# GT-RIPL/robo-vln

Measured on AMD Instinct MI355X. Metric: policy env-steps/sec (batched act()) at 256x256 RGB-D, 80-tok instr, higher is better.
Workload: dtype fp16 (range-calibrated fp16 storage and MFMA in BERT, both trunks and the cross-modal block; fp32 accumulate, fp32 recurrent state; DESIGN.md section 5); 1 GPU; BASELINE.json configs[1]: full HCM act() (hi->argmax->lo), 256x256 RGB-D, L=80, VLA N=1, LSTM-512; per_gpu_batch=64, global_batch=64, parallelism=single GPU

## Files before the change

### include/hcm.h

```cpp
#ifndef HCM_H
#define HCM_H

#include <stdint.h>

#ifdef __cplusplus
extern "C" {
#endif

typedef struct hcm_ctx* hcm_handle;

enum hcm_status {
    HCM_OK = 0,
    HCM_ERR_ARG = -1,
    HCM_ERR_STATE = -2,
    HCM_ERR_KEY = -3,
    HCM_ERR_SHAPE = -4,
    HCM_ERR_HIP = -5,
    HCM_ERR_UNSUPPORTED = -6,
    HCM_ERR_NOMEM = -7
};

enum hcm_dtype { HCM_F32 = 0, HCM_BF16 = 1, HCM_I32 = 2, HCM_I64 = 3, HCM_U8 = 4, HCM_F16 = 5 };
enum hcm_model { HCM_HIGH = 0, HCM_LOW = 1, HCM_CMA = 2 ,
                 HCM_S2S = 3  };
// ... 162 lines not shown


int hcm_debug_enable_taps(hcm_handle h, int enable);
int hcm_debug_get_tap(hcm_handle h, const char* name, float* host_out, int64_t capacity,
                      int64_t* n_out, int64_t* shape_out);
int hcm_debug_igemm_prof(uint64_t* out8, int reset);
int hcm_debug_gemm256_prof(uint64_t* out1024, int reset);
int hcm_debug_marks(hcm_handle h, uint64_t* out256, char* names, int names_cap);

int hcm_op_conv2d(const void* x, const void* w_ohwi, const float* bias, const void* residual, void* y,
                  int dtype, int B, int H, int W, int Cin, int Cout, int KH, int KW, int stride, int pad,
                  int act, void* stream);
int hcm_op_conv2d_gn(const void* x, const void* w_ohwi, const float* gamma, const float* beta, const void* residual, void* y,
                     int dtype, int B, int H, int W, int Cin, int Cout, int KH, int KW, int stride, int pad, int groups, float eps,
                     int relu, void* stream);
int hcm_op_bottleneck_tail(const void* x, const void* w2, const float* b2, const void* w3, const float* b3, const void* identity,
                           void* y, int dtype, int B, int H, int W, int C1, int stride, void* stream);
int hcm_op_bottleneck_tail_next(const void* x, const void* w2, const float* b2, const void* w3, const float* b3, const void* identity,
                                void* y, const void* w1, const float* b1, void* o1, int dtype, int B, int H, int W, int C1, int stride,
                                int CN, void* stream);
int hcm_op_bottleneck_tail_ds(const void* x, const void* w2, const float* b2, const void* w3ds, const float* b3ds, const void* xd,
                              void* y, const void* w1, const float* b1, void* o1, int dtype, int B, int H, int W, int stride,
                              void* stream);
int hcm_op_conv2d_gn_large(const void* x, const void* w_ohwi, const float* gamma, const float* beta, const void* residual, void* y,
                           int dtype, int B, int H, int W, int Cin, int Cout, int KH, int KW, int stride, int pad, int groups, float eps,
                           int relu, void* stream);
int hcm_op_stem_conv(const void* x, int x_dtype, const void* w, const float* bias, void* y, int dtype, int B, int H, int W, int C,
                     int Cout, int KH, int KW, int stride, int pad, int K, int Kp, int rowrun, float scale, int act, void* stream);
int hcm_op_stem_conv_packed(const void* x, int x_dtype, const void* w, const float* bias, void* y, int dtype, int B, int H, int W,
                            int Cout, float scale, int act, void* scratch, void* stream);
int hcm_op_stem_conv_packed_pool(const void* x, int x_dtype, const void* w, const float* bias, void* y, int dtype, int B, int H, int W,
                                 int Cout, float scale, void* scratch, void* half_map, void* stream);
int hcm_op_stem_pool_fused(const void* x, int x_dtype, const void* w, const float* bias, void* y, int dtype, int B, int H, int W,
                           int Cout, float scale, void* scratch, void* stream);
int hcm_op_stem_pool_fused_red(const void* x, int x_dtype, const void* w, const float* bias, void* y, int dtype, int B, int H, int W,
                               int Cout, float scale, void* scratch, const void* w1, const float* b1, void* o1, void* stream);
int64_t hcm_op_stem_scratch_bytes(int B, int H, int W);
int hcm_op_depth_conv8x8s4(const float* depth, const void* w, const float* bias, void* y, int dtype, int B, int H, int act, void* scratch,
                           void* stream);
int hcm_op_simplecnn3(const float* depth, const void* w0, const float* b0, const void* w1_frag, const float* b1, const void* w2_frag, const float* b2,
                      void* y, int dtype, int B, int H, void* stream);
int hcm_op_linear(const void* x, const void* w, const float* bias, const void* residual, void* y,
                  int dtype, int M, int N, int K, int act, int out_f32, void* stream);
int hcm_op_vla_layer(const void* q, const void* I, const void* const* kv, const int* Lk, const void* const* att, void* const* out, float* const* pooled,
                     int ld_pool, const void* wo, const float* bo, const void* w1, const float* b1, const void* w2, const float* b2, const float* g1,
                     const float* be1, const float* g2, const float* be2, const int32_t* lens, int dtype, int B, int L, int d_ff, int streams,
// ... 32 lines not shown
```

### robo-vln_amd/_lib.py

```python
import ctypes as C
import os

_HERE = os.path.dirname(os.path.abspath(__file__))
LIB_PATH = os.path.join(_HERE, "libhcm_dev.so" if os.environ.get("HCM_DEV_LIB", "0") not in ("", "0") else "libhcm.so")

HCM_F32, HCM_BF16, HCM_I32, HCM_I64, HCM_U8, HCM_F16 = 0, 1, 2, 3, 4, 5
HCM_HIGH, HCM_LOW, HCM_CMA, HCM_S2S = 0, 1, 2, 3
HCM_ENC_RESNET, HCM_ENC_SIMPLECNN = 0, 1
HCM_LSTM, HCM_GRU = 0, 1
(HCM_NUM_RECURRENT_LAYERS, HCM_HIDDEN_SIZE, HCM_NUM_ACTIONS, HCM_RECORD_WIDTH, HCM_WORKSPACE_BYTES,
 HCM_WEIGHT_BYTES, HCM_MAX_BATCH, HCM_GRAPH_LAUNCHES, HCM_EAGER_LAUNCHES, HCM_FP16_FALLBACK, HCM_CALIB_MAX_BERT, HCM_CALIB_MAX_DEPTH,
 HCM_CALIB_NONFINITE, HCM_CALIB_MAX_RGB, HCM_CALIB_MAX_VLA, HCM_STEP_NONFINITE, HCM_RANGE_FOLD, HCM_GATHER_JOINED) = range(18)
PRECISIONS = {"fp32": HCM_F32, "fp16": HCM_F16, "bf16": HCM_BF16}
ACT_NONE, ACT_RELU, ACT_GELU = 0, 1, 2
HCM_ACT_REUSE_INSTRUCTION = 1
HCM_ACT_HOST_FRAMES = 2
HCM_ACT_CHAIN_GRAPHS = 4

STATUS_EXC = {-1: ValueError, -2: RuntimeError, -3: KeyError, -4: ValueError, -5: RuntimeError, -6: ValueError,
              -7: MemoryError}


class HcmConfigStruct(C.Structure):
    _fields_ = [(n, C.c_int32) for n in (
# ... 50 lines not shown
                             C.c_void_p, C.c_void_p, C.c_void_p, C.c_void_p, C.c_void_p, C.c_void_p, C.c_int, C.c_void_p]),
    "hcm_comm_unique_id": (C.c_int, [C.c_void_p]),
    "hcm_comm_init": (C.c_int, [C.c_void_p, C.c_void_p, C.c_int, C.c_int]),
    "hcm_comm_abort": (C.c_int, [C.c_void_p]),
    "hcm_gather_poison": (C.c_int, [C.c_void_p, C.c_int, C.c_void_p, C.c_void_p, C.c_void_p]),
    "hcm_act_gather": (C.c_int, [C.c_void_p, C.c_void_p, C.c_int, C.c_void_p, C.c_void_p, C.c_int, C.c_void_p, C.c_int, C.c_int,
                                 C.c_void_p, C.c_void_p, C.c_void_p, C.c_void_p, C.c_void_p, C.c_void_p, C.c_int, C.c_void_p, C.c_void_p]),
    "hcm_refresh_instruction": (C.c_int, [C.c_void_p, C.c_void_p, C.c_int, C.c_void_p, C.c_int, C.c_int, C.POINTER(C.c_int32), C.c_int, C.c_void_p]),
    "hcm_calibrate": (C.c_int, [C.c_void_p, C.c_void_p, C.c_int, C.c_void_p, C.c_void_p, C.c_int, C.c_int, C.c_int, C.c_void_p]),
    "hcm_release_host_weights": (C.c_int, [C.c_void_p]),
    "hcm_query": (C.c_int, [C.c_void_p, C.c_int, C.POINTER(C.c_int64)]),
    "hcm_guard_poll": (C.c_int, [C.c_void_p, C.c_void_p, C.POINTER(C.c_int64)]),
    "hcm_last_error": (C.c_char_p, [C.c_void_p]),
    "hcm_destroy": (None, [C.c_void_p]),
    "hcm_debug_enable_taps": (C.c_int, [C.c_void_p, C.c_int]),
    "hcm_debug_get_tap": (C.c_int, [C.c_void_p, C.c_char_p, C.c_void_p, C.c_int64, C.POINTER(C.c_int64), C.POINTER(C.c_int64)]),
    "hcm_debug_igemm_prof": (C.c_int, [C.POINTER(C.c_uint64), C.c_int]),
    "hcm_debug_gemm256_prof": (C.c_int, [C.POINTER(C.c_uint64), C.c_int]),
    "hcm_debug_marks": (C.c_int, [C.c_void_p, C.POINTER(C.c_uint64), C.c_char_p, C.c_int]),
    "hcm_op_conv2d": (C.c_int, [C.c_void_p] * 5 + [C.c_int] * 11 + [C.c_void_p]),
    "hcm_op_bottleneck_tail": (C.c_int, [C.c_void_p] * 7 + [C.c_int] * 6 + [C.c_void_p]),
    "hcm_op_bottleneck_tail_next": (C.c_int, [C.c_void_p] * 10 + [C.c_int] * 7 + [C.c_void_p]),
    "hcm_op_bottleneck_tail_ds": (C.c_int, [C.c_void_p] * 10 + [C.c_int] * 5 + [C.c_void_p]),
    "hcm_op_conv2d_gn": (C.c_int, [C.c_void_p] * 6 + [C.c_int] * 11 + [C.c_float, C.c_int, C.c_void_p]),
    "hcm_op_conv2d_gn_large": (C.c_int, [C.c_void_p] * 6 + [C.c_int] * 11 + [C.c_float, C.c_int, C.c_void_p]),
    "hcm_op_stem_conv": (C.c_int, [C.c_void_p, C.c_int, C.c_void_p, C.c_void_p, C.c_void_p] + [C.c_int] * 13 + [C.c_float, C.c_int, C.c_void_p]),
    "hcm_op_stem_conv_packed": (C.c_int, [C.c_void_p, C.c_int, C.c_void_p, C.c_void_p, C.c_void_p] + [C.c_int] * 5 + [C.c_float, C.c_int, C.c_void_p, C.c_void_p]),
    "hcm_op_stem_pool_fused": (C.c_int, [C.c_void_p, C.c_int, C.c_void_p, C.c_void_p, C.c_void_p] + [C.c_int] * 5 + [C.c_float, C.c_void_p, C.c_void_p]),
    "hcm_op_stem_pool_fused_red": (C.c_int, [C.c_void_p, C.c_int, C.c_void_p, C.c_void_p, C.c_void_p] + [C.c_int] * 5 + [C.c_float] + [C.c_void_p] * 5),
    "hcm_op_stem_conv_packed_pool": (C.c_int, [C.c_void_p, C.c_int, C.c_void_p, C.c_void_p, C.c_void_p] + [C.c_int] * 5 + [C.c_float, C.c_void_p, C.c_void_p, C.c_void_p]),
    "hcm_op_depth_conv8x8s4": (C.c_int, [C.c_void_p] * 4 + [C.c_int] * 4 + [C.c_void_p, C.c_void_p]),
    "hcm_op_stem_scratch_bytes": (C.c_int64, [C.c_int] * 3),
    "hcm_op_linear": (C.c_int, [C.c_void_p] * 5 + [C.c_int] * 6 + [C.c_void_p]),
    "hcm_op_linear_impl": (C.c_int, [C.c_void_p] * 5 + [C.c_int] * 7 + [C.c_void_p]),
    "hcm_op_vla_layer": (C.c_int, [C.c_void_p] * 7 + [C.c_int] + [C.c_void_p] * 11 + [C.c_int] * 5 + [C.c_void_p]),
    "hcm_op_vla_layer_frag": (C.c_int, [C.c_void_p] * 7 + [C.c_int] + [C.c_void_p] * 11 + [C.c_int] * 5 + [C.c_void_p]),
    "hcm_op_attention": (C.c_int, [C.c_void_p] * 4 + [C.c_int] * 9 + [C.c_void_p]),
    "hcm_op_simplecnn3": (C.c_int, [C.c_void_p] * 8 + [C.c_int] * 3 + [C.c_void_p]),
    "hcm_op_pack_frag": (C.c_int, [C.c_void_p, C.c_void_p, C.c_int, C.c_int, C.c_int, C.c_void_p]),
    "hcm_op_bert_attn_block": (C.c_int, [C.c_void_p] * 9 + [C.c_int] * 3 + [C.c_void_p, C.c_float, C.c_void_p]),
    "hcm_op_layernorm": (C.c_int, [C.c_void_p] * 5 + [C.c_int] * 3 + [C.c_float, C.c_void_p]),
    "hcm_op_layernorm_post": (C.c_int, [C.c_void_p] * 5 + [C.c_int, C.c_void_p] + [C.c_int] * 3 + [C.c_float, C.c_void_p]),
    "hcm_op_groupnorm": (C.c_int, [C.c_void_p] * 4 + [C.c_int] * 5 + [C.c_float, C.c_int, C.c_void_p]),
    "hcm_op_conv2d_gn_pool": (C.c_int, [C.c_void_p] * 5 + [C.c_int] * 11 + [C.c_float, C.c_void_p]),
    "hcm_op_conv2d_gn_res2": (C.c_int, [C.c_void_p] * 9 + [C.c_int] * 9 + [C.c_float, C.c_int, C.c_void_p]),
    "hcm_op_val_loss": (C.c_int, [C.c_void_p] * 7 + [C.c_int] * 3 + [C.c_void_p]),
# ... 33 lines not shown
```

### robo-vln_amd/csrc/api.cpp

```cpp
#include <chrono>
#include <cmath>
#include <cstdlib>
#include <cstring>
#include <stdexcept>
#include <string>

#include "model.h"

namespace hcm {
void build_spec_high(hcm_ctx* ctx);
void build_spec_low(hcm_ctx* ctx);
void prepare_high(hcm_ctx* ctx);
void prepare_low(hcm_ctx* ctx);
void build_spec_cma(hcm_ctx* ctx);
void prepare_cma(hcm_ctx* ctx);
void run_refresh_instruction(hcm_ctx* ctx, const void* ids, int ids_dt, int B, const int32_t* idx, int n);
void run_cma(hcm_ctx* ctx, const void* rgb, int rgb_dt, const float* depth, const void* ids, int ids_dt, int B, const float* h_in,
             const float* mask, float* out, float* stop, float* h_out);
void build_spec_s2s(hcm_ctx* ctx);
void prepare_s2s(hcm_ctx* ctx);
void run_s2s(hcm_ctx* ctx, const void* rgb, int rgb_dt, const float* depth, const void* ids, int ids_dt, int B, int Bi, const float* h_in,
             const float* mask, float* out, float* stop, float* progress, float* h_out, int T = 1);
void comm_destroy(hcm_ctx* ctx);
void run_step(hcm_ctx* ctx, bool do_hi, bool do_lo, const void* rgb, int rgb_dt, const float* depth, const void* ids, int ids_dt,
// ... 1121 lines not shown
    return op_rc(launch_bneck23(b, op_dt(dtype), (hipStream_t)stream));
}
int hcm_op_bottleneck_tail_next(const void* x, const void* w2, const float* b2, const void* w3, const float* b3, const void* identity,
                                void* y, const void* w1, const float* b1, void* o1, int dtype, int B, int H, int W, int C1, int stride,
                                int CN, void* stream) {
    Bneck23 b;
    b.x = x; b.w2 = w2; b.b2 = b2; b.w3 = w3; b.b3 = b3; b.res = identity; b.y = y;
    b.B = B; b.H = H; b.W = W; b.C1 = C1; b.stride = stride;
    b.w1 = w1; b.b1 = b1; b.o1 = o1; b.CN = CN;
    if (!w1) return HCM_ERR_ARG;
    return op_rc(launch_bneck23(b, op_dt(dtype), (hipStream_t)stream));
}
int hcm_op_bottleneck_tail_ds(const void* x, const void* w2, const float* b2, const void* w3ds, const float* b3ds, const void* xd,
                              void* y, const void* w1, const float* b1, void* o1, int dtype, int B, int H, int W, int stride,
                              void* stream) {
    if (!xd || !w1) return HCM_ERR_ARG;
    Bneck23 b;
    b.x = x; b.w2 = w2; b.b2 = b2; b.w3 = w3ds; b.b3 = b3ds; b.y = y;
    b.B = B; b.H = H; b.W = W; b.C1 = 64; b.stride = stride;
    b.w1 = w1; b.b1 = b1; b.o1 = o1; b.CN = 64;
    b.xd = xd; b.xdC = 64; b.KD = 1;
    return op_rc(launch_bneck23(b, op_dt(dtype), (hipStream_t)stream));
}
int hcm_op_conv2d_gn(const void* x, const void* w_ohwi, const float* gamma, const float* beta, const void* residual, void* y,
                     int dtype, int B, int H, int W, int Cin, int Cout, int KH, int KW, int stride, int pad, int groups, float eps,
                     int relu, void* stream) {
    if (groups < 1 || Cout % groups) return HCM_ERR_ARG;
    IGemm g;
    g.x = x; g.w = w_ohwi; g.res = residual; g.y = y;
    g.B = B; g.H = H; g.W = W; g.Cin = Cin; g.xC = Cin;
    g.Ho = (H + 2 * pad - KH) / stride + 1; g.Wo = (W + 2 * pad - KW) / stride + 1;
    g.KH = KH; g.KW = KW; g.stride = stride; g.pad = pad;
    g.M = B * g.Ho * g.Wo; g.N = Cout; g.K = KH * KW * Cin; g.Kp = g.K; g.ldy = Cout; g.ldr = Cout; g.act = relu ? ACT_RELU : ACT_NONE;
    g.gn_gamma = gamma; g.gn_beta = beta; g.gn_cg = Cout / groups; g.gn_hw = g.Ho * g.Wo; g.gn_eps = eps;
    return op_rc(launch_igemm(g, op_dt(dtype), (hipStream_t)stream));
}
int hcm_op_stem_conv(const void* x, int x_dtype, const void* w, const float* bias, void* y, int dtype, int B, int H, int W, int C, int Cout,
                     int KH, int KW, int stride, int pad, int K, int Kp, int rowrun, float scale, int act, void* stream) {
    IGemm g;
    g.x = x; g.w = w; g.bias = bias; g.y = y;
    g.B = B; g.H = H; g.W = W; g.Cin = C; g.xC = C;
    g.Ho = (H + 2 * pad - KH) / stride + 1; g.Wo = (W + 2 * pad - KW) / stride + 1;
    g.KH = KH; g.KW = KW; g.stride = stride; g.pad = pad;
    g.M = B * g.Ho * g.Wo; g.N = Cout; g.K = K; g.Kp = Kp; g.ldy = Cout; g.ldr = Cout; g.act = act;
    g.x_src_dt = x_dtype == HCM_U8 ? DT_U8 : x_dtype == HCM_F32 ? DT_F32 : op_dt(x_dtype);
    g.x_scale = scale; g.x_rowrun = rowrun;
// ... 271 lines not shown
```

### robo-vln_amd/csrc/forward.cpp

```cpp
#include <cstdio>
#include <cstdlib>
#include <stdexcept>

#include "model.h"

namespace hcm {

int depth_final_spatial(const hcm_config& c);
int depth_compress_channels(const hcm_config& c);

struct Act { void* p = nullptr; int B = 0, H = 0, W = 0, C = 0; };

struct Fwd {
    hcm_ctx* ctx;
    Arena& ar;
    hipStream_t s;
    int dt;
    size_t esz;
    bool dry;

    explicit Fwd(hcm_ctx* c) : ctx(c), ar(c->arena), s(c->stream), dt(c->dt_vla), esz(dt_size(c->dt_vla)), dry(c->arena.dry) {}

    void use(int d) { dt = d; esz = dt_size(d); }

// ... 374 lines not shown
            int fr[3], nf = 0;
            if (pre >= 0) fr[nf++] = pre;
            for (int i = 0; i < 4; ++i) if (i != xi && i != pre) fr[nf++] = i;
            if (nf != 3) throw std::runtime_error("trunk slot rotation: expected three free activation slots");
            if (xpend.valid && xpend.res && slot[fr[0]] == xpend.res) std::swap(fr[0], fr[1]);
            void* sa = slot[fr[0]]; void* sb = slot[fr[1]]; void* sc = slot[fr[2]];
            if (xpend.valid && xpend.res && sa == xpend.res) throw std::runtime_error("trunk slot rotation: c1 would overwrite a pending identity");
            const int Ho2 = (x.H + 2 - 3) / b.stride + 1, Wo2 = (x.W + 2 - 3) / b.stride + 1;
            Act o1{sa, B, x.H, x.W, CO(b.c1)};
            const bool have_o1 = pre >= 0;
            pre = -1;
            Pending p1, p2;
            if (have_o1) {}
            else if (t.gn) {
                if (xpend.valid) { xpend.writeback = true; pend_in = xpend; xpend.valid = false; }
                defer_out = &p1;
                conv_gn(b.c1, x, sa, 1, 0, nullptr, b.n1, G, true, x.H, x.W);
            }
            else conv(b.c1, x, sa, 1, 0, nullptr, ACT_RELU, x.H, x.W);
            static const bool no_tail = dev_env("HCM_NO_BNECK_FUSE") != nullptr;
            static const bool no_next = dev_env("HCM_NO_BNECK_NEXT") != nullptr;
            static const bool no_256 = dev_env("HCM_NO_BNECK256") != nullptr;
            static const bool force_256 = dev_env("HCM_FORCE_BNECK256") != nullptr;
            const BottleneckW* nb = bi + 1 < t.blocks.size() ? &t.blocks[bi + 1] : nullptr;
            static const int next_only = dev_env("HCM_BNECK_NEXT_ONLY") ? atoi(dev_env("HCM_BNECK_NEXT_ONLY")) : 0;
            const bool next = nb && !no_next && (!next_only || next_only == b.c2.Cout) && nb->c1.KH == 1 && nb->c1.KW == 1 && nb->c1.Cin == b.c3.Cout && nb->c1.Kp == nb->c1.Cin &&
                              nb->c1.bias && nb->c1.groups == b.c2.groups && nb->c1.dt == b.c2.dt &&
                              ((nb->c1.Cout == b.c2.Cout && (nb->c1.Cout == 64 || nb->c1.Cout == 128 || nb->c1.Cout == 256)) || (b.c2.Cout == 64 && nb->c1.Cout == 128));
            const long tiles256 = (long)b.c2.groups * (((long)B * ((x.H + 2 - 3) / b.stride + 1) * ((x.W + 2 - 3) / b.stride + 1) + 127) / 128);
            const bool c1_ok = b.c2.Cout == 64 || b.c2.Cout == 128 || (b.c2.Cout == 256 && next && !no_256 && (tiles256 >= 192 || force_256));
            if (!t.gn && !no_tail && (b.c2.dt == DT_BF16 || b.c2.dt == DT_F16) && c1_ok && b.c2.KH == 3 &&
                b.c2.Cin == b.c2.Cout && b.c2.Kp == 9 * b.c2.Cin && b.c3.Cout == 4 * b.c2.Cout && b.c3.Kp == b.c2.Cout && b.c2.bias && b.c3.bias &&
                b.c3.groups == b.c2.groups) {
                const void* idt = x.p;
                static const bool no_dsfold = dev_env("HCM_NO_BNECK_DSFOLD") != nullptr;
                const bool dsfold = b.has_ds && !no_dsfold && next && b.c3ds.w && b.c2.Cout == 64 && nb->c1.Cout == 64 && b.ds.Cin == 64 &&
                                    b.c3ds.Kp == 128 && b.c3ds.groups == b.c2.groups && x.C == b.c2.groups * 64;
                if (b.has_ds && !dsfold) {
                    conv(b.ds, x, sb, b.stride, 0, nullptr, ACT_NONE, Ho2, Wo2);
                    idt = sb;
                }
                const int pre_slot = (b.has_ds && !dsfold) ? xi : fr[1];
                if (!dry) {
                    Bneck23 q;
                    q.x = sa; q.w2 = b.c2.w; q.b2 = b.c2.bias; q.w3 = b.c3.w; q.b3 = b.c3.bias; q.res = idt; q.y = sc;
                    q.B = B; q.H = x.H; q.W = x.W; q.C1 = b.c2.Cout; q.xC = o1.C; q.stride = b.stride;
                    q.ldy = q.ldr = CO(b.c3);
                    if (b.c2.groups > 1) {
                        q.groups = b.c2.groups; q.g_x = b.c2.Cin; q.g_w2 = (long long)b.c2.Cout * b.c2.Kp; q.g_b2 = b.c2.Cout;
                        q.g_w3 = (long long)b.c3.Cout * b.c3.Kp; q.g_b3 = b.c3.Cout; q.g_y = b.c3.Cout;
                    }
                    if (next) {
                        q.w1 = nb->c1.w; q.b1 = nb->c1.bias; q.o1 = slot[pre_slot]; q.CN = nb->c1.Cout; q.ldo = CO(nb->c1);
                        if (b.c2.groups > 1) { q.g_w1 = (long long)nb->c1.Cout * nb->c1.Kp; q.g_b1 = nb->c1.Cout; q.g_o1 = nb->c1.Cout; }
                    }
                    if (dsfold) {
                        q.w3 = b.c3ds.w; q.b3 = b.c3ds.bias; q.res = nullptr;
                        q.xd = x.p; q.xdC = x.C; q.KD = 1;
                        if (b.c2.groups > 1) { q.g_w3 = (long long)b.c3ds.Cout * b.c3ds.Kp; q.g_xd = 64; }
                    }
                    ck(launch_bneck23(q, b.c2.dt, s), "bottleneck tail");
                    calib_check(sc, b.c2.dt, B * Ho2 * Wo2, CO(b.c3), CO(b.c3));
                }
                if (next) pre = pre_slot;
                x = Act{sc, B, Ho2, Wo2, CO(b.c3)};
                xi = fr[2];
                ++bidx;
                if (bidx == 3 || bidx == 7 || bidx == 13 || bidx == 16) {
                    tap(tapname + "_layer" + std::to_string(bidx == 3 ? 1 : bidx == 7 ? 2 : bidx == 13 ? 3 : 4), x.p, true, {B, x.H, x.W, x.C});
                    mark(tapname + ".layer" + std::to_string(bidx == 3 ? 1 : bidx == 7 ? 2 : bidx == 13 ? 3 : 4) + "_end");
                }
                continue;
            }
            Act o2{sb, B, Ho2, Wo2, CO(b.c2)};
            if (t.gn) {
                pend_in = p1; p1.valid = false;
                defer_out = &p2;
                conv_gn(b.c2, o1, sb, b.stride, 1, nullptr, b.n2, G, true, Ho2, Wo2);
            }
            else conv(b.c2, o1, sb, b.stride, 1, nullptr, ACT_RELU, Ho2, Wo2);
            const void* idt = x.p;
            Pending pds;
// ... 1146 lines not shown
```

### robo-vln_amd/csrc/igemm.hip

```cpp
#include <cstdio>
#include <cstdlib>
#include <cstring>
#include <type_traits>
#include <vector>
#include <algorithm>
#include <mutex>
#include <string>
#include <unordered_map>
#include "kernels.h"
#include "dev.h"

namespace hcm {

typedef float f32x4 __attribute__((ext_vector_type(4)));
typedef __bf16 bf16x8 __attribute__((ext_vector_type(8)));

struct IGemmDev {
    const char* x; const char* w; const float* bias; const char* res; char* y;
    int B, H, W, Cin, xC, Ho, Wo, KH, KW, stride, pad;
    int stride_w;
    int M, N, K, Kp, ldy, ldr, act, out_f32;
    int image_epi;
    int res_f32;
    int cin_shift, kw_rcp, tilesM, tilesN, map;
// ... 3065 lines not shown
            g_choice[key] = choice;
        } else {
            choice = heuristic_choice(d, dt);
        }
    }
    static const bool log_shapes = dev_env("HCM_IGEMM_LOG") != nullptr;
    if (log_shapes) {
        static std::unordered_map<std::string, int> seen;
        std::lock_guard<std::mutex> l(g_choice_mu);
        if (seen.emplace(key, choice).second)
            fprintf(stderr, "[igemm] dt=%d M=%d N=%d K=%d groups=%d KHxKW=%dx%d stride=%d res=%d -> choice %d\n", dt, d.M, d.N, d.K, d.groups, d.KH, d.KW,
                    d.stride, d.res != nullptr, choice);
    }
    return launch_dt(d, dt, choice, s);
}


constexpr int kHaloRing = 5, kHaloRingD = 5;

hipError_t launch_bneck23(const Bneck23& b, int dt, hipStream_t s) {
    if (dt != DT_BF16 && dt != DT_F16) return hipErrorInvalidValue;
    if ((b.C1 != 64 && b.C1 != 128 && b.C1 != 256) || (!b.res && !b.xd) || !b.b2 || !b.b3 || b.stride < 1) return hipErrorInvalidValue;
    if (b.C1 == 256 && (!b.w1 || b.CN != 256 || b.xd)) return hipErrorInvalidValue;
    if (b.xd && (b.C1 != 64 || b.KD != 1 || !b.w1 || b.CN != 64 || (b.xdC % 8))) return hipErrorInvalidValue;
    const int C3 = 4 * b.C1;
    const int ldy = b.ldy ? b.ldy : C3, ldr = b.ldr ? b.ldr : C3, xC = b.xC ? b.xC : b.C1;
    if ((ldy % 8) || (ldr % 8) || (xC % 8)) return hipErrorInvalidValue;
    BneckDev q;
    IGemmDev& d = q.a;
    memset((void*)&q, 0, sizeof(q));
    d.x = (const char*)b.x; d.w = (const char*)b.w2; d.bias = b.b2;
    d.B = b.B; d.H = b.H; d.W = b.W; d.Cin = b.C1; d.xC = xC;
    d.Ho = (b.H + 2 - 3) / b.stride + 1; d.Wo = (b.W + 2 - 3) / b.stride + 1;
    d.KH = 3; d.KW = 3; d.stride = b.stride; d.stride_w = b.stride; d.pad = 1;
    d.M = b.B * d.Ho * d.Wo; d.N = b.C1; d.K = 9 * b.C1; d.Kp = 9 * b.C1;
    d.cin_shift = b.C1 == 64 ? 6 : b.C1 == 128 ? 7 : 8;
    d.kw_rcp = (65536 + 3 - 1) / 3;
    d.groups = b.groups > 1 ? b.groups : 1;
    d.g_x = b.g_x; d.g_w = b.g_w2; d.g_b = b.g_b2;
    {
        const size_t xb = (((size_t)d.B * d.H * d.W - 1) * d.xC + d.Cin) * 2, wb = (size_t)d.N * d.Kp * 2, w3b = (size_t)C3 * b.C1 * 2;
        if (xb >= 0xFFFFFFF0ull) return hipErrorInvalidValue;
        d.x_bytes = (unsigned)xb; d.w_bytes = (unsigned)wb; q.w3_bytes = (unsigned)w3b;
    }
    q.w3 = (const char*)b.w3; q.b3 = b.b3; q.res = (const char*)b.res; q.y = (char*)b.y;
    q.C3 = C3; q.Kp3 = b.C1 + (b.xd ? b.KD * 64 : 0); q.ldy3 = ldy; q.ldr3 = ldr;
    q.w3_bytes = (unsigned)((size_t)C3 * q.Kp3 * 2);
    q.g_w3 = b.g_w3; q.g_b3 = b.g_b3; q.g_y3 = b.g_y;
    const int BM = b.C1 == 128 ? 64 : 128;
    const int KT1 = b.C1 / 64;
    if (b.w1) {
        if (!b.b1 || !b.o1 || (b.CN != 64 && b.CN != 128 && b.CN != 256) || (b.C1 == 128 && b.CN != 128) || ((b.C1 == 256) != (b.CN == 256))) return hipErrorInvalidValue;
        const int ldo = b.ldo ? b.ldo : b.CN;
        if (ldo % 8) return hipErrorInvalidValue;
        Bneck231Dev qq;
        qq.t = q;
        qq.w1 = (const char*)b.w1; qq.b1 = b.b1; qq.o1 = (char*)b.o1; qq.ldo = ldo;
        qq.w1_bytes = (unsigned)((size_t)b.CN * C3 * 2);
        qq.g_w1 = b.g_w1; qq.g_b1 = b.g_b1; qq.g_o1 = b.g_o1;
        qq.xd = nullptr; qq.xdC = 0; qq.xd_bytes = 0; qq.g_xd = 0;
        qq.xcd_tiles = 0;
        if (b.xd) {
            const size_t xdb = (((size_t)d.B * d.H * d.W - 1) * b.xdC + b.KD * 64) * 2;
            if (xdb >= 0xFFFFFFF0ull) return hipErrorInvalidValue;
            qq.xd = (const char*)b.xd; qq.xdC = b.xdC; qq.xd_bytes = (unsigned)xdb; qq.g_xd = b.g_xd;
            const int BMd = 64;
            static const bool image_d = dev_env("HCM_BNECK_IMAGE") != nullptr;
            size_t ldsd = image_d ? (size_t)2 * BMd * 128 + (size_t)2 * 64 * 128 + (64 * 132 * 4 / 2 + 1024) + (size_t)BMd * 128 + (size_t)b.CN * 128
                                  : (size_t)2 * BMd * 128 + (size_t)2 * 64 * 128 + (size_t)BMd * 128 + (size_t)2 * b.CN * 128 + (size_t)(4 * b.C1 + b.CN) * 4;
            const size_t ringd = 3 * (size_t)(BMd + b.C1) * 128;
            if (ringd > ldsd) ldsd = ringd;
            const void* fd = image_d ? (dt == DT_BF16 ? reinterpret_cast<const void*>(bneck231_kernel<bf16, 64, 64, 64, 1>) : reinterpret_cast<const void*>(bneck231_kernel<f16, 64, 64, 64, 1>))
                                     : (dt == DT_BF16 ? reinterpret_cast<const void*>(bneck231r_kernel<bf16, 64, 64, 64, 1>) : reinterpret_cast<const void*>(bneck231r_kernel<f16, 64, 64, 64, 1>));
            static const bool no_halo_d = dev_env("HCM_NO_BNECK_HALO") != nullptr;
            static const bool no_big_d = dev_env("HCM_NO_BNECK_DS128") != nullptr;
            if (!image_d && !no_halo_d && !no_big_d && b.stride == 1 && d.W % 16 == 0 && 128 % d.W == 0 && (d.Ho * d.Wo) % 128 == 0) {
                const size_t halo = (size_t)((((128 / d.W + 2) * (d.W + 2)) + 7) & ~7) * 128 + (size_t)kHaloRing * 64 * 128;
                size_t lds = (size_t)2 * 128 * 128 + (size_t)2 * 64 * 128 + (size_t)128 * 128 + (size_t)b.CN * 128 + (size_t)(4 * b.C1 + b.CN) * 4;
                if (halo > lds) lds = halo;
                if (lds <= 80 * 1024) {
                    const void* fb = dt == DT_BF16 ? reinterpret_cast<const void*>(bneck231r_kernel<bf16, 128, 64, 64, 1, false, kHaloRing, 1>)
                                                   : reinterpret_cast<const void*>(bneck231r_kernel<f16, 128, 64, 64, 1, false, kHaloRing, 1>);
                    hipError_t eb = hipFuncSetAttribute(fb, hipFuncAttributeMaxDynamicSharedMemorySize, 160 * 1024);
                    if (eb != hipSuccess) return eb;
                    void* ab[] = {&qq};
                    return hipLaunchKernel(fb, dim3((d.M + 127) / 128, d.groups), dim3(512), ab, lds, s);
                }
            }
// ... 8 lines not shown
            }
            hipError_t ed = hipFuncSetAttribute(fd, hipFuncAttributeMaxDynamicSharedMemorySize, 160 * 1024);
            if (ed != hipSuccess) return ed;
            void* ad[] = {&qq};
            return hipLaunchKernel(fd, dim3((d.M + BMd - 1) / BMd, d.groups), dim3(512), ad, ldsd, s);
        }
        if (b.C1 == 256) {
            const size_t lb = (size_t)KT1 * BM * 128 + (size_t)KT1 * 64 * 128 + (size_t)BM * 128 + (size_t)b.CN * 128 + (size_t)(4 * b.C1 + b.CN) * 4;
            const size_t ra = 3 * (size_t)(BM + b.C1) * 128;
            const size_t lds256 = lb > ra ? lb : ra;
            if (lds256 > 160 * 1024) return hipErrorInvalidValue;
            const void* f2 = dt == DT_BF16 ? reinterpret_cast<const void*>(bneck231r_kernel<bf16, 128, 256, 256, 0, false, 0, 1>)
                                           : reinterpret_cast<const void*>(bneck231r_kernel<f16, 128, 256, 256, 0, false, 0, 1>);
            hipError_t e2 = hipFuncSetAttribute(f2, hipFuncAttributeMaxDynamicSharedMemorySize, 160 * 1024);
            if (e2 != hipSuccess) return e2;
            void* a2[] = {&qq};
            static const bool no_xcd = dev_env("HCM_NO_BNECK_XCD") != nullptr;
            if (d.groups == 2 && !no_xcd) {
                const int tiles = (d.M + BM - 1) / BM;
                qq.xcd_tiles = tiles;
                return hipLaunchKernel(f2, dim3(((tiles + 3) / 4) * 8, 1), dim3(512), a2, lds256, s);
            }
            return hipLaunchKernel(f2, dim3((d.M + BM - 1) / BM, d.groups), dim3(512), a2, lds256, s);
        }
        static const bool image = dev_env("HCM_BNECK_IMAGE") != nullptr;
        size_t lds1 = image ? (size_t)KT1 * BM * 128 + (size_t)KT1 * 64 * 128 + (64 * 132 * 4 / 2 + 1024) + (size_t)BM * 128 + (size_t)b.CN * 128
                            : (size_t)KT1 * BM * 128 + (size_t)KT1 * 64 * 128 + (size_t)BM * 128 + (size_t)2 * b.CN * 128 + (size_t)(4 * b.C1 + b.CN) * 4;
        const size_t ring1 = 3 * (size_t)(BM + b.C1) * 128;
        if (ring1 > lds1) lds1 = ring1;
        const void* f1;
        if (image) {
            if (dt == DT_BF16) f1 = b.C1 == 128 ? reinterpret_cast<const void*>(bneck231_kernel<bf16, 64, 128, 128>)
                                  : b.CN == 64 ? reinterpret_cast<const void*>(bneck231_kernel<bf16, 128, 64, 64>) : reinterpret_cast<const void*>(bneck231_kernel<bf16, 128, 64, 128>);
            else f1 = b.C1 == 128 ? reinterpret_cast<const void*>(bneck231_kernel<f16, 64, 128, 128>)
                    : b.CN == 64 ? reinterpret_cast<const void*>(bneck231_kernel<f16, 128, 64, 64>) : reinterpret_cast<const void*>(bneck231_kernel<f16, 128, 64, 128>);
        } else {
            if (dt == DT_BF16) f1 = b.C1 == 128 ? reinterpret_cast<const void*>(bneck231r_kernel<bf16, 64, 128, 128>)
                                  : b.CN == 64 ? reinterpret_cast<const void*>(bneck231r_kernel<bf16, 128, 64, 64>) : reinterpret_cast<const void*>(bneck231r_kernel<bf16, 128, 64, 128>);
            else f1 = b.C1 == 128 ? reinterpret_cast<const void*>(bneck231r_kernel<f16, 64, 128, 128>)
                    : b.CN == 64 ? reinterpret_cast<const void*>(bneck231r_kernel<f16, 128, 64, 64>) : reinterpret_cast<const void*>(bneck231r_kernel<f16, 128, 64, 128>);
        }
        static const bool no_halo = dev_env("HCM_NO_BNECK_HALO") != nullptr;
        static const bool bm64 = dev_env("HCM_BNECK128_BM64") != nullptr;
        if (!image && !no_halo && !bm64 && b.C1 == 128 && b.CN == 128 && b.stride == 1 && d.W % 16 == 0 && 128 % d.W == 0 && (d.Ho * d.Wo) % 128 == 0 &&
            (long)d.groups * (d.M / 128) >= 192) {
            const size_t halo = (size_t)KT1 * ((((128 / d.W + 2) * (d.W + 2)) + 7) & ~7) * 128 + (size_t)kHaloRing * 8192;
// ... 308 lines not shown
```

### robo-vln_amd/csrc/weights.cpp

```cpp
#include <cmath>
#include <cstdlib>
#include <cstring>
#include <stdexcept>

#include "model.h"

namespace hcm {

static const int RESNET50_BLOCKS[4] = {3, 4, 6, 3};

struct SpecB {
    std::map<std::string, HostTensor>& m;
    void add(const std::string& k, Shape s) { m[k].shape = std::move(s); }
    void conv(const std::string& k, int co, int ci, int kh, int kw) { add(k, {co, ci, kh, kw}); }
    void linear(const std::string& p, int o, int i) { add(p + ".weight", {o, i}); add(p + ".bias", {o}); }
    void norm(const std::string& p, int c) { add(p + ".weight", {c}); add(p + ".bias", {c}); }
    void bn(const std::string& p, int c) {
        norm(p, c); add(p + ".running_mean", {c}); add(p + ".running_var", {c}); add(p + ".num_batches_tracked", {});
    }
};

static void spec_tv_resnet50(SpecB& s, const std::string& pre, bool with_fc) {
    s.conv(pre + "conv1.weight", 64, 3, 7, 7); s.bn(pre + "bn1", 64);
    int inpl = 64;
// ... 370 lines not shown
    c.w = up.typed(r, dt);
    c.bias = up.f32(bias);
    return c;
}

static ConvW make_c3ds(hcm_ctx* ctx, int dt, Uploader& up, const std::vector<int>& models, const std::string& p);
static TrunkW make_tv_trunk(hcm_ctx* ctx, Uploader& up, int model, const std::string& pre) {
    TrunkW t;
    const int dt = ctx->dt_rgb;
    t.gn = false;
    t.cin1 = 3;
    t.conv1 = make_conv_bn(ctx, dt, up, model, pre + "conv1.weight", pre + "bn1", true);
    t.conv1_rowrun = make_stem_rowrun(ctx, dt, up, model, pre + "conv1.weight", pre + "bn1");
    if (dt != DT_F32) t.conv1_packed = make_stem_packed(ctx, dt, up, model, pre + "conv1.weight", pre + "bn1");
    for (int li = 0; li < 4; ++li)
        for (int bi = 0; bi < RESNET50_BLOCKS[li]; ++bi) {
            const std::string p = pre + "layer" + std::to_string(li + 1) + "." + std::to_string(bi) + ".";
            BottleneckW b;
            b.stride = (li > 0 && bi == 0) ? 2 : 1;
            b.c1 = make_conv_bn(ctx, dt, up, model, p + "conv1.weight", p + "bn1");
            b.c2 = make_conv_bn(ctx, dt, up, model, p + "conv2.weight", p + "bn2");
            b.c3 = make_conv_bn(ctx, dt, up, model, p + "conv3.weight", p + "bn3");
            if (bi == 0) { b.has_ds = true; b.ds = make_conv_bn(ctx, dt, up, model, p + "downsample.0.weight", p + "downsample.1"); }
            if (li == 0 && bi == 0 && dt != DT_F32) b.c3ds = make_c3ds(ctx, dt, up, {model}, p);
            t.blocks.push_back(b);
        }
    t.out_c = 2048;
    return t;
}

static ConvW make_depth_stem_packed(int dt, Uploader& up, const std::vector<const HostTensor*>& ws, float fold = 1.f) {
    ConvW c;
    c.dt = dt;
    c.fold = fold; c.calib_pos = 0;
    const int Co = (int)ws[0]->shape[0];
    c.Cout = Co * (int)ws.size(); c.Cin = 1; c.KH = 7; c.KW = 7; c.K = 56; c.Kp = 64;
    std::vector<float> r((size_t)c.Cout * c.Kp, 0.f);
    for (size_t g = 0; g < ws.size(); ++g)
        for (int o = 0; o < Co; ++o)
            for (int kh = 0; kh < 7; ++kh)
                for (int kw = 0; kw < 7; ++kw) r[((size_t)g * Co + o) * c.Kp + kh * 8 + kw] = ws[g]->f[((size_t)o * 7 + kh) * 7 + kw] * fold;
    c.w = up.typed(r, dt);
    return c;
}

static int gn_pos(int block, int which) { return 1 + 4 * block + which; }
static float gn_fold(hcm_ctx* ctx, int pos) { return ctx->dt_depth == DT_F16 ? ctx->depth_fold[pos] : 1.f; }
// ... 192 lines not shown
                        rk[((size_t)g * Co + o) * packed.Kp + kh * 32 + kw * 4 + ci] = v;
                    }
    }
    plain.w = up.typed(rp, dt); rowrun.w = up.typed(rr, dt);
    plain.bias = up.f32(bias_all); rowrun.bias = up.f32(bias_all);
    if (dt != DT_F32) { packed.w = up.typed(rk, dt); packed.bias = up.f32(bias_all); }
}
static TrunkW make_tv_trunk_pair(hcm_ctx* ctx, Uploader& up, const std::string& pre) {
    TrunkW t;
    const int dt = ctx->dt_rgb;
    t.gn = false;
    t.pair = true;
    t.cin1 = 3;
    make_stem_pair(ctx, dt, up, pre + "conv1.weight", pre + "bn1", t.conv1, t.conv1_rowrun, t.conv1_packed);
    for (int li = 0; li < 4; ++li)
        for (int bi = 0; bi < RESNET50_BLOCKS[li]; ++bi) {
            const std::string p = pre + "layer" + std::to_string(li + 1) + "." + std::to_string(bi) + ".";
            BottleneckW b;
            b.stride = (li > 0 && bi == 0) ? 2 : 1;
            b.c1 = make_conv_bn_pair(ctx, dt, up, p + "conv1.weight", p + "bn1");
            b.c2 = make_conv_bn_pair(ctx, dt, up, p + "conv2.weight", p + "bn2");
            b.c3 = make_conv_bn_pair(ctx, dt, up, p + "conv3.weight", p + "bn3");
            if (bi == 0) { b.has_ds = true; b.ds = make_conv_bn_pair(ctx, dt, up, p + "downsample.0.weight", p + "downsample.1"); }
            if (li == 0 && bi == 0 && dt != DT_F32) b.c3ds = make_c3ds(ctx, dt, up, {HCM_HIGH, HCM_LOW}, p);
            t.blocks.push_back(b);
        }
    t.out_c = 2048;
    return t;
}

static SimpleCnnW make_simple_cnn(hcm_ctx* ctx, int dt, Uploader& up, int model, const std::string& pre, int cin, int h, int w) {
    SimpleCnnW s;
    s.cin = cin; s.h = h; s.w = w; s.h3 = simple_cnn_out_hw(h); s.w3 = simple_cnn_out_hw(w);
    s.c0 = make_conv(dt, up, T_(ctx, model, pre + "cnn.0.weight"), nullptr, &T_(ctx, model, pre + "cnn.0.bias").f);
    if (dt != DT_F32 && (cin == 1 || cin == 3) && w % 4 == 0) {
        const HostTensor& w0 = T_(ctx, model, pre + "cnn.0.weight");
        const int cp = cin == 3 ? 4 : 1, KR = 8 * cp;
        ConvW c;
        c.dt = dt; c.Cout = (int)w0.shape[0]; c.Cin = cin; c.KH = 8; c.KW = 8; c.K = 8 * KR; c.Kp = c.K;
        std::vector<float> r((size_t)c.Cout * c.Kp, 0.f);
        for (int o = 0; o < c.Cout; ++o)
            for (int ci = 0; ci < cin; ++ci)
                for (int kh = 0; kh < 8; ++kh)
                    for (int kw = 0; kw < 8; ++kw)
                        r[(size_t)o * c.Kp + kh * KR + kw * cp + ci] = w0.f[(((size_t)o * cin + ci) * 8 + kh) * 8 + kw];
        c.w = up.typed(r, dt);
        c.bias = up.f32(T_(ctx, model, pre + "cnn.0.bias").f);
// ... 371 lines not shown
```

Baseline: 15540 env-steps/s.

## Extend fused bottleneck tail to layer2: downsample fold and 128->256 next-conv fusion

Extends the fused bottleneck conv2+conv3(+next conv1) kernel to the ResNet layer2 stage. The layer2 first block can now fold its strided downsample conv into the conv3 GEMM (KD=4, concatenated weights built for layer<=1). A new path fuses the layer2-last-block tail with layer3's first conv1 (128->256), with halo and ring LDS variants. This removes separate downsample and conv1 launches and their intermediate round trips through global memory. In exchange it needs larger LDS footprints, which may lower occupancy. It also exposes a test op entry point.

Result: faster. 15840 env-steps/s (median of 6 runs) (+1.9%).

```diff
diff --git a/include/hcm.h b/include/hcm.h
--- a/include/hcm.h
+++ b/include/hcm.h
@@ -208,6 +208,9 @@
 int hcm_op_bottleneck_tail_ds(const void* x, const void* w2, const float* b2, const void* w3ds, const float* b3ds, const void* xd,
                               void* y, const void* w1, const float* b1, void* o1, int dtype, int B, int H, int W, int stride,
                               void* stream);
+int hcm_op_bottleneck_stage(const void* x, const void* w2, const float* b2, const void* w3, const float* b3, const void* identity,
+                            const void* xd, void* y, const void* w1, const float* b1, void* o1, int dtype, int B, int H, int W, int C1,
+                            int stride, int CN, int KD, int groups, void* stream);
 int hcm_op_conv2d_gn_large(const void* x, const void* w_ohwi, const float* gamma, const float* beta, const void* residual, void* y,
                            int dtype, int B, int H, int W, int Cin, int Cout, int KH, int KW, int stride, int pad, int groups, float eps,
                            int relu, void* stream);
diff --git a/robo-vln_amd/_lib.py b/robo-vln_amd/_lib.py
--- a/robo-vln_amd/_lib.py
+++ b/robo-vln_amd/_lib.py
@@ -96,6 +96,7 @@
     "hcm_op_bottleneck_tail": (C.c_int, [C.c_void_p] * 7 + [C.c_int] * 6 + [C.c_void_p]),
     "hcm_op_bottleneck_tail_next": (C.c_int, [C.c_void_p] * 10 + [C.c_int] * 7 + [C.c_void_p]),
     "hcm_op_bottleneck_tail_ds": (C.c_int, [C.c_void_p] * 10 + [C.c_int] * 5 + [C.c_void_p]),
+    "hcm_op_bottleneck_stage": (C.c_int, [C.c_void_p] * 11 + [C.c_int] * 9 + [C.c_void_p]),
     "hcm_op_conv2d_gn": (C.c_int, [C.c_void_p] * 6 + [C.c_int] * 11 + [C.c_float, C.c_int, C.c_void_p]),
     "hcm_op_conv2d_gn_large": (C.c_int, [C.c_void_p] * 6 + [C.c_int] * 11 + [C.c_float, C.c_int, C.c_void_p]),
     "hcm_op_stem_conv": (C.c_int, [C.c_void_p, C.c_int, C.c_void_p, C.c_void_p, C.c_void_p] + [C.c_int] * 13 + [C.c_float, C.c_int, C.c_void_p]),
diff --git a/robo-vln_amd/csrc/api.cpp b/robo-vln_amd/csrc/api.cpp
--- a/robo-vln_amd/csrc/api.cpp
+++ b/robo-vln_amd/csrc/api.cpp
@@ -1167,6 +1167,23 @@
     b.xd = xd; b.xdC = 64; b.KD = 1;
     return op_rc(launch_bneck23(b, op_dt(dtype), (hipStream_t)stream));
 }
+int hcm_op_bottleneck_stage(const void* x, const void* w2, const float* b2, const void* w3, const float* b3, const void* identity,
+                            const void* xd, void* y, const void* w1, const float* b1, void* o1, int dtype, int B, int H, int W, int C1,
+                            int stride, int CN, int KD, int groups, void* stream) {
+    if (!w1 || groups < 1 || KD < 0 || (xd != nullptr) != (KD > 0) || (xd && identity)) return HCM_ERR_ARG;
+    const int C3 = 4 * C1, K3 = C1 + 64 * KD;
+    Bneck23 b;
+    b.x = x; b.w2 = w2; b.b2 = b2; b.w3 = w3; b.b3 = b3; b.res = identity; b.y = y;
+    b.B = B; b.H = H; b.W = W; b.C1 = C1; b.stride = stride; b.xC = groups * C1; b.ldy = b.ldr = groups * C3;
+    b.w1 = w1; b.b1 = b1; b.o1 = o1; b.CN = CN; b.ldo = groups * CN;
+    b.xd = xd; b.xdC = xd ? groups * 64 * KD : 0; b.KD = KD;
+    if (groups > 1) {
+        b.groups = groups; b.g_x = C1; b.g_w2 = (long long)C1 * 9 * C1; b.g_b2 = C1;
+        b.g_w3 = (long long)C3 * K3; b.g_b3 = C3; b.g_y = C3;
+        b.g_w1 = (long long)CN * C3; b.g_b1 = CN; b.g_o1 = CN; b.g_xd = 64 * KD;
+    }
+    return op_rc(launch_bneck23(b, op_dt(dtype), (hipStream_t)stream));
+}
 int hcm_op_conv2d_gn(const void* x, const void* w_ohwi, const float* gamma, const float* beta, const void* residual, void* y,
                      int dtype, int B, int H, int W, int Cin, int Cout, int KH, int KW, int stride, int pad, int groups, float eps,
                      int relu, void* stream) {
diff --git a/robo-vln_amd/csrc/forward.cpp b/robo-vln_amd/csrc/forward.cpp
--- a/robo-vln_amd/csrc/forward.cpp
+++ b/robo-vln_amd/csrc/forward.cpp
@@ -420,11 +420,13 @@
             static const bool no_next = dev_env("HCM_NO_BNECK_NEXT") != nullptr;
             static const bool no_256 = dev_env("HCM_NO_BNECK256") != nullptr;
             static const bool force_256 = dev_env("HCM_FORCE_BNECK256") != nullptr;
+            static const bool no_next256 = dev_env("HCM_NO_BNECK_NEXT256") != nullptr;
             const BottleneckW* nb = bi + 1 < t.blocks.size() ? &t.blocks[bi + 1] : nullptr;
             static const int next_only = dev_env("HCM_BNECK_NEXT_ONLY") ? atoi(dev_env("HCM_BNECK_NEXT_ONLY")) : 0;
             const bool next = nb && !no_next && (!next_only || next_only == b.c2.Cout) && nb->c1.KH == 1 && nb->c1.KW == 1 && nb->c1.Cin == b.c3.Cout && nb->c1.Kp == nb->c1.Cin &&
                               nb->c1.bias && nb->c1.groups == b.c2.groups && nb->c1.dt == b.c2.dt &&
-                              ((nb->c1.Cout == b.c2.Cout && (nb->c1.Cout == 64 || nb->c1.Cout == 128 || nb->c1.Cout == 256)) || (b.c2.Cout == 64 && nb->c1.Cout == 128));
+                              ((nb->c1.Cout == b.c2.Cout && (nb->c1.Cout == 64 || nb->c1.Cout == 128 || nb->c1.Cout == 256)) || (b.c2.Cout == 64 && nb->c1.Cout == 128) ||
+                               (b.c2.Cout == 128 && nb->c1.Cout == 256 && !no_next256));
             const long tiles256 = (long)b.c2.groups * (((long)B * ((x.H + 2 - 3) / b.stride + 1) * ((x.W + 2 - 3) / b.stride + 1) + 127) / 128);
             const bool c1_ok = b.c2.Cout == 64 || b.c2.Cout == 128 || (b.c2.Cout == 256 && next && !no_256 && (tiles256 >= 192 || force_256));
             if (!t.gn && !no_tail && (b.c2.dt == DT_BF16 || b.c2.dt == DT_F16) && c1_ok && b.c2.KH == 3 &&
@@ -432,8 +434,11 @@
                 b.c3.groups == b.c2.groups) {
                 const void* idt = x.p;
                 static const bool no_dsfold = dev_env("HCM_NO_BNECK_DSFOLD") != nullptr;
-                const bool dsfold = b.has_ds && !no_dsfold && next && b.c3ds.w && b.c2.Cout == 64 && nb->c1.Cout == 64 && b.ds.Cin == 64 &&
-                                    b.c3ds.Kp == 128 && b.c3ds.groups == b.c2.groups && x.C == b.c2.groups * 64;
+                static const bool no_dsfold128 = dev_env("HCM_NO_BNECK_DSFOLD128") != nullptr;
+                const int dsC = b.has_ds ? b.ds.Cin : 0;
+                const bool dsfold = b.has_ds && !no_dsfold && next && b.c3ds.w && nb->c1.Cout == b.c2.Cout &&
+                                    ((b.c2.Cout == 64 && dsC == 64) || (b.c2.Cout == 128 && dsC == 256 && !no_dsfold128)) &&
+                                    b.c3ds.Kp == b.c2.Cout + dsC && b.c3ds.groups == b.c2.groups && x.C == b.c2.groups * dsC;
                 if (b.has_ds && !dsfold) {
                     conv(b.ds, x, sb, b.stride, 0, nullptr, ACT_NONE, Ho2, Wo2);
                     idt = sb;
@@ -454,8 +459,8 @@
                     }
                     if (dsfold) {
                         q.w3 = b.c3ds.w; q.b3 = b.c3ds.bias; q.res = nullptr;
-                        q.xd = x.p; q.xdC = x.C; q.KD = 1;
-                        if (b.c2.groups > 1) { q.g_w3 = (long long)b.c3ds.Cout * b.c3ds.Kp; q.g_xd = 64; }
+                        q.xd = x.p; q.xdC = x.C; q.KD = dsC / 64;
+                        if (b.c2.groups > 1) { q.g_w3 = (long long)b.c3ds.Cout * b.c3ds.Kp; q.g_xd = dsC; }
                     }
                     ck(launch_bneck23(q, b.c2.dt, s), "bottleneck tail");
                     calib_check(sc, b.c2.dt, B * Ho2 * Wo2, CO(b.c3), CO(b.c3));
diff --git a/robo-vln_amd/csrc/igemm.hip b/robo-vln_amd/csrc/igemm.hip
--- a/robo-vln_amd/csrc/igemm.hip
+++ b/robo-vln_amd/csrc/igemm.hip
@@ -3111,7 +3111,7 @@
     if (dt != DT_BF16 && dt != DT_F16) return hipErrorInvalidValue;
     if ((b.C1 != 64 && b.C1 != 128 && b.C1 != 256) || (!b.res && !b.xd) || !b.b2 || !b.b3 || b.stride < 1) return hipErrorInvalidValue;
     if (b.C1 == 256 && (!b.w1 || b.CN != 256 || b.xd)) return hipErrorInvalidValue;
-    if (b.xd && (b.C1 != 64 || b.KD != 1 || !b.w1 || b.CN != 64 || (b.xdC % 8))) return hipErrorInvalidValue;
+    if (b.xd && (!b.w1 || (b.xdC % 8) || !((b.C1 == 64 && b.KD == 1 && b.CN == 64) || (b.C1 == 128 && b.KD == 4 && b.CN == 128)))) return hipErrorInvalidValue;
     const int C3 = 4 * b.C1;
     const int ldy = b.ldy ? b.ldy : C3, ldr = b.ldr ? b.ldr : C3, xC = b.xC ? b.xC : b.C1;
     if ((ldy % 8) || (ldr % 8) || (xC % 8)) return hipErrorInvalidValue;
@@ -3139,7 +3139,7 @@
     const int BM = b.C1 == 128 ? 64 : 128;
     const int KT1 = b.C1 / 64;
     if (b.w1) {
-        if (!b.b1 || !b.o1 || (b.CN != 64 && b.CN != 128 && b.CN != 256) || (b.C1 == 128 && b.CN != 128) || ((b.C1 == 256) != (b.CN == 256))) return hipErrorInvalidValue;
+        if (!b.b1 || !b.o1 || (b.CN != 64 && b.CN != 128 && b.CN != 256) || (b.C1 == 128 && b.CN == 64) || (b.C1 == 64 && b.CN == 256) || (b.C1 == 256 && b.CN != 256)) return hipErrorInvalidValue;
         const int ldo = b.ldo ? b.ldo : b.CN;
         if (ldo % 8) return hipErrorInvalidValue;
         Bneck231Dev qq;
@@ -3153,6 +3153,18 @@
             const size_t xdb = (((size_t)d.B * d.H * d.W - 1) * b.xdC + b.KD * 64) * 2;
             if (xdb >= 0xFFFFFFF0ull) return hipErrorInvalidValue;
             qq.xd = (const char*)b.xd; qq.xdC = b.xdC; qq.xd_bytes = (unsigned)xdb; qq.g_xd = b.g_xd;
+            if (b.C1 == 128) {
+                const size_t lp = (size_t)2 * (2 + b.KD) * 64 * 128 + (size_t)64 * 128 + (size_t)2 * b.CN * 128 + (size_t)(4 * b.C1 + b.CN) * 4;
+                const size_t rp = 3 * (size_t)(64 + b.C1) * 128;
+                const size_t ldsp = lp > rp ? lp : rp;
+                if (ldsp > 160 * 1024) return hipErrorInvalidValue;
+                const void* fp = dt == DT_BF16 ? reinterpret_cast<const void*>(bneck231r_kernel<bf16, 64, 128, 128, 4>)
+                                               : reinterpret_cast<const void*>(bneck231r_kernel<f16, 64, 128, 128, 4>);
+                hipError_t ep = hipFuncSetAttribute(fp, hipFuncAttributeMaxDynamicSharedMemorySize, 160 * 1024);
+                if (ep != hipSuccess) return ep;
+                void* ap[] = {&qq};
+                return hipLaunchKernel(fp, dim3((d.M + 63) / 64, d.groups), dim3(512), ap, ldsp, s);
+            }
             const int BMd = 64;
             static const bool image_d = dev_env("HCM_BNECK_IMAGE") != nullptr;
             size_t ldsd = image_d ? (size_t)2 * BMd * 128 + (size_t)2 * 64 * 128 + (64 * 132 * 4 / 2 + 1024) + (size_t)BMd * 128 + (size_t)b.CN * 128
@@ -3207,6 +3219,41 @@
                 return hipLaunchKernel(f2, dim3(((tiles + 3) / 4) * 8, 1), dim3(512), a2, lds256, s);
             }
             return hipLaunchKernel(f2, dim3((d.M + BM - 1) / BM, d.groups), dim3(512), a2, lds256, s);
+        }
+        if (b.C1 == 128 && b.CN == 256) {
+            static const bool no_halo2 = dev_env("HCM_NO_BNECK_HALO") != nullptr;
+            static const bool bm64_2 = dev_env("HCM_BNECK128_BM64") != nullptr;
+            const void* f3 = nullptr;
+            size_t lds3 = 0;
+            int BM3 = 64;
+            if (!no_halo2 && !bm64_2 && b.stride == 1 && d.W % 16 == 0 && 128 % d.W == 0 && (d.Ho * d.Wo) % 128 == 0 && (long)d.groups * (d.M / 128) >= 192) {
+                const size_t halo = (size_t)KT1 * ((((128 / d.W + 2) * (d.W + 2)) + 7) & ~7) * 128 + (size_t)kHaloRing * 8192;
+                size_t lds = (size_t)KT1 * 128 * 128 + (size_t)KT1 * 64 * 128 + (size_t)128 * 128 + (size_t)b.CN * 128 + (size_t)(4 * b.C1 + b.CN) * 4;
+                if (halo > lds) lds = halo;
+                if (lds <= 112 * 1024) {
+                    BM3 = 128; lds3 = lds;
+                    f3 = dt == DT_BF16 ? reinterpret_cast<const void*>(bneck231r_kernel<bf16, 128, 128, 256, 0, false, kHaloRing, 1>)
+                                       : reinterpret_cast<const void*>(bneck231r_kernel<f16, 128, 128, 256, 0, false, kHaloRing, 1>);
+                }
+            }
+            if (!f3) {
+                lds3 = (size_t)KT1 * 64 * 128 + (size_t)KT1 * 64 * 128 + (size_t)64 * 128 + (size_t)b.CN * 128 + (size_t)(4 * b.C1 + b.CN) * 4;
+                const size_t halo = (size_t)KT1 * ((((64 / d.W + 2) * (d.W + 2)) + 7) & ~7) * 128 + (size_t)kHaloRing * 8192;
+                if (!no_halo2 && b.stride == 1 && d.W % 16 == 0 && 64 % d.W == 0 && (d.Ho * d.Wo) % 64 == 0 && halo <= 80 * 1024) {
+                    if (halo > lds3) lds3 = halo;
+                    f3 = dt == DT_BF16 ? reinterpret_cast<const void*>(bneck231r_kernel<bf16, 64, 128, 256, 0, false, kHaloRing, 1>)
+                                       : reinterpret_cast<const void*>(bneck231r_kernel<f16, 64, 128, 256, 0, false, kHaloRing, 1>);
+                } else {
+                    const size_t ring3 = 3 * (size_t)(64 + b.C1) * 128;
+                    if (ring3 > lds3) lds3 = ring3;
+                    f3 = dt == DT_BF16 ? reinterpret_cast<const void*>(bneck231r_kernel<bf16, 64, 128, 256, 0, false, 0, 1>)
+                                       : reinterpret_cast<const void*>(bneck231r_kernel<f16, 64, 128, 256, 0, false, 0, 1>);
+                }
+            }
+            hipError_t e3 = hipFuncSetAttribute(f3, hipFuncAttributeMaxDynamicSharedMemorySize, 160 * 1024);
+            if (e3 != hipSuccess) return e3;
+            void* a3[] = {&qq};
+            return hipLaunchKernel(f3, dim3((d.M + BM3 - 1) / BM3, d.groups), dim3(512), a3, lds3, s);
         }
         static const bool image = dev_env("HCM_BNECK_IMAGE") != nullptr;
         size_t lds1 = image ? (size_t)KT1 * BM * 128 + (size_t)KT1 * 64 * 128 + (64 * 132 * 4 / 2 + 1024) + (size_t)BM * 128 + (size_t)b.CN * 128
diff --git a/robo-vln_amd/csrc/weights.cpp b/robo-vln_amd/csrc/weights.cpp
--- a/robo-vln_amd/csrc/weights.cpp
+++ b/robo-vln_amd/csrc/weights.cpp
@@ -416,7 +416,7 @@
             b.c2 = make_conv_bn(ctx, dt, up, model, p + "conv2.weight", p + "bn2");
             b.c3 = make_conv_bn(ctx, dt, up, model, p + "conv3.weight", p + "bn3");
             if (bi == 0) { b.has_ds = true; b.ds = make_conv_bn(ctx, dt, up, model, p + "downsample.0.weight", p + "downsample.1"); }
-            if (li == 0 && bi == 0 && dt != DT_F32) b.c3ds = make_c3ds(ctx, dt, up, {model}, p);
+            if (li <= 1 && bi == 0 && dt != DT_F32) b.c3ds = make_c3ds(ctx, dt, up, {model}, p);
             t.blocks.push_back(b);
         }
     t.out_c = 2048;
@@ -655,7 +655,7 @@
             b.c2 = make_conv_bn_pair(ctx, dt, up, p + "conv2.weight", p + "bn2");
             b.c3 = make_conv_bn_pair(ctx, dt, up, p + "conv3.weight", p + "bn3");
             if (bi == 0) { b.has_ds = true; b.ds = make_conv_bn_pair(ctx, dt, up, p + "downsample.0.weight", p + "downsample.1"); }
-            if (li == 0 && bi == 0 && dt != DT_F32) b.c3ds = make_c3ds(ctx, dt, up, {HCM_HIGH, HCM_LOW}, p);
+            if (li <= 1 && bi == 0 && dt != DT_F32) b.c3ds = make_c3ds(ctx, dt, up, {HCM_HIGH, HCM_LOW}, p);
             t.blocks.push_back(b);
         }
     t.out_c = 2048;
```
